# HoangChuongNguyen/cope-nerf

Measured on AMD Instinct MI355X. Metric: rays/sec (train step incl. backward) at 4096 rays × 128 samples, higher is better.
Workload: dtype fp32; 1 GPU; C2: synthetic scene, 4096 rays x 128 samples (64 coarse + 4x16 importance) per GPU, fp32, fixed poses, full train step (fwd + losses + bwd + Adam); rays_per_gpu=4096, samples_per_ray=128, global_rays=4096, hip_graph=False, parallelism=single

## Files before the change

### cope-nerf_amd/copenerf/_lib.py

```python
from __future__ import annotations

import ctypes
import os
import threading

import numpy as np

_HERE = os.path.dirname(os.path.abspath(__file__))
LIB_NAME = "libcopenerf.so"
LIB_PATH = os.environ.get("COPENERF_LIB", os.path.join(_HERE, LIB_NAME))

ABI_VERSION = 21

c_f32p = ctypes.c_void_p
c_i32 = ctypes.c_int32
c_i64 = ctypes.c_int64
c_f32 = ctypes.c_float
c_ptr = ctypes.c_void_p

EPI_STORE = 0
EPI_SOFTPLUS = 1
EPI_RELU = 2
EPI_MUL = 3
EPI_TANGENT = 4
EPI_BWD_SOFTPLUS = 5
EPI_BWD_RELU = 6
EPI_SOFTPLUS_HEAD = 8


class WnJob(ctypes.Structure):
    _fields_ = [("v", c_ptr), ("g", c_ptr), ("w", c_ptr), ("dw", c_ptr), ("dv", c_ptr), ("dg", c_ptr),
                ("rows", c_i32), ("cols", c_i32)]


class LinearDesc(ctypes.Structure):
# ... 320 lines not shown
```

### cope-nerf_amd/copenerf/ops.py

```python
from __future__ import annotations

import ctypes
import math

import torch

from . import _lib
from ._lib import (EPI_BWD_RELU, EPI_BWD_SOFTPLUS, EPI_MUL, EPI_RELU, EPI_SOFTPLUS, EPI_SOFTPLUS_HEAD,
                   EPI_STORE, EPI_TANGENT)

SQRT2 = float(math.sqrt(2.0))


class KernelTimer:

    def __init__(self, detail=False):
        self.records = []
        self.detail = detail
        self.symbols = {}

    def start(self):
        e = torch.cuda.Event(enable_timing=True)
        e.record()
        return e
# ... 125 lines not shown
        rows, cols = (src.shape[1], src.shape[0]) if transpose else (src.shape[0], src.shape[1])
        j = _lib.PackJob()
        j.src, j.dst = src.data_ptr(), dst.data_ptr()
        j.src_ld = src.stride(0)
        x6 = fmt == "bf16x6"
        d_rows, d_cols = (dst.shape[1], 16 * dst.shape[0]) if x6 else (dst.shape[0], dst.shape[1])
        j.dst_ld = d_rows if x6 else d_cols
        j.rows, j.cols = rows, cols
        j.r0, j.r1 = r0, d_rows if r1 is None else r1
        j.c0, j.c1 = c0, d_cols if c1 is None else c1
        j.transpose, j.format = int(transpose), FORMATS[fmt]
        self.jobs.append(j)
        self.keep.append(src)
        return dst

    def run(self):
        if self.jobs:
            arr = (_lib.PackJob * len(self.jobs))(*self.jobs)
            _lib.check(_lib.load().cn_pack_weights(arr, len(self.jobs), _stream()), "cn_pack_weights")
        self.jobs, self.keep = [], []


_TILE_TAGS = {"4, 2, 2, 4, 16, 1, 2": "sq", "4, 2, 1, 4, 32, 1, 2": "tall", "4, 2, 2, 2, 32, 1, 2": "wide",
              "2, 2, 2, 2, 16, 2, 2": "t128", "4, 1, 1, 2, 16, 2, 2": "t1", "4, 2, 2, 4, 32, 1, 2": "sq",
              "2, 2, 2, 2, 64, 2, 1": "t128", "4, 1, 1, 2, 64, 2, 1": "t1"}


def kernel_name(query, d) -> str:
    buf = ctypes.create_string_buffer(256)
    n = query(d, buf, 256)
    if n < 0:
        raise RuntimeError(f"kernel name query failed ({n}): {_lib.load().cn_last_error().decode()}")
    return buf.value.decode()


def _tile_tag(name, tile):
    args = name[name.index("<") + 1:].split(", ")[:7]
    return _TILE_TAGS.get(", ".join(args), tile)


def linear(A, B, N, K, out0, epilogue, *, bias=None, A2=None, K1=None, rowv=None, colv=None, aux0=None,
           aux1=None, aux2=None, out_split=None, nsplit=None, nzero=None, adiv=1.0, odiv=1.0, beta=100.0,
           threshold=20.0, aux_beta=0.0, aux2_scale=0.0, tile=None, M=None, kalg=None, out1=None, head_w=None,
           head_b=None, head_out=None, head_idx=None, out0_b=None, out1_b=None):
    x6 = B.dim() == 3
    if x6 and (B.dtype != torch.bfloat16 or B.shape[2] != 48 or not B.is_contiguous()):
# ... 961 lines not shown
```

### cope-nerf_amd/csrc/cn_gemm.hip

```cpp
#include "cn_mfma.h"

#include <algorithm>
#include <type_traits>
#include <cstdlib>

namespace cn {

struct LinearArgs {
    const float* A;
    const float* A2;
    const float* B;
    const float* bias;
    const float* rowv;
    const float* colv;
    const float* aux0;
    const float* aux1;
    const float* aux2;
    float* out0;
    float* out1;
    float* out_split;
    int lda, lda2, ldb, ld_aux0, ld_aux1, ld_aux2, ld_out0, ld_out1, ld_split;
    int M, N, K, K1, nzero, nsplit, n_tiles_m, n_tiles_n;
    float inv_adiv, inv_odiv, beta, threshold;
    float aux_c;
    float aux2_scale;
    const float* head_w;
    const float* head_b;
    float* head_out;
    const int* head_idx;
    int flags;
    bf16_t* out0_b;
    bf16_t* out1_b;
    int ld_out0_b, ld_out1_b;
};


constexpr int kTblCols = 512;

#ifndef CN_DMA_A_NT
#define CN_DMA_A_NT 0
#endif
template <int WM, int WN, int TM, int TN, int BK, int OCC, int DEPTH, int EPI, bool ROWV, int MODE_>
__global__ void __launch_bounds__(64 * WM * WN, OCC * WM * WN / 4) linear_kernel(LinearArgs p) {
    constexpr int MODE = MODE_ & 3;
    constexpr bool ABF = (MODE_ & 4) != 0;
    constexpr bool AUX0B = (MODE_ & 8) != 0 && (EPI == CN_EPI_BWD_RELU || EPI == CN_EPI_MUL || EPI == CN_EPI_TANGENT ||
                                                EPI == CN_EPI_BWD_SOFTPLUS);
    constexpr bool AUX12B = (MODE_ & 8) != 0 && EPI == CN_EPI_BWD_SOFTPLUS;
    static_assert(!ABF || MODE == 1, "bf16 A images only in the bf16 MFMA mode");
    constexpr bool AX6 = (MODE_ & 16) != 0;
    static_assert(!AX6 || (MODE == 2 && BK == 16), "bf16x6 A images: 16-deep stages of the bf16x6 mode");
    constexpr int NT = 64 * WM * WN;
    const float* const cA = p.A;
    const float* const cB = p.B;
    float* const cOut0 = p.out0;
    const int cN = p.N, cNzero = p.nzero;
    const float cInvOdiv = p.inv_odiv;
    constexpr int BM = 32 * TM * WM;
    constexpr int BN = 32 * TN * WN;
    constexpr bool BF = MODE != 0;
    constexpr int NPL = MODE == 2 ? 3 : 1;
    constexpr int LS = (BF ? NPL * BK / 2 : BK) + (MODE == 2 && BK == 16 ? 12 : 4);
    constexpr int EPA = ABF ? 8 : 4;
    constexpr int ESA = ABF ? 2 : 4;
    constexpr int KC4 = BK / EPA;
    static_assert(NT % KC4 == 0, "staging rows");
    constexpr int RSTEP = NT / KC4;
    constexpr int KCB = BF ? NPL * BK / 8 : BK / 4;
    constexpr int RSTEPB = MODE == 2 ? 1 : NT / KCB;
    static_assert(BM % RSTEP == 0 && (MODE == 2 || (NT % KCB == 0 && BN % RSTEPB == 0)), "tile/thread mismatch");
    constexpr int ALD = AX6 ? (BM * 6 + NT - 1) / NT : BM / RSTEP;
    constexpr int BLD = MODE == 2 ? (BN * KCB + NT - 1) / NT : BN / RSTEPB;
    constexpr int ESZB = BF ? 2 : 4;
    constexpr int PIECES_PL = BK / 8;
    constexpr int CS = BN + 4;
    constexpr int LDS_FLOATS = 2 * BM * LS + 2 * BN * LS;
    constexpr int NPART = (BM * CS <= LDS_FLOATS) ? 1 : ((BM / 2) * CS <= LDS_FLOATS ? 2 : 4);
    static_assert((BM / NPART) * CS <= LDS_FLOATS, "C tile slab must fit in the staging LDS");
    constexpr int PROWS = BM / NPART;

    constexpr bool kHead = EPI == CN_EPI_SOFTPLUS_HEAD;
    constexpr bool kBias = EPI == CN_EPI_STORE || EPI == CN_EPI_SOFTPLUS || EPI == CN_EPI_RELU || kHead;
    constexpr bool kColv = ROWV || kHead;
    constexpr int TBLC = kHead ? 256 : kTblCols;
    constexpr int TBL = (kBias ? TBLC : 0) + (kColv ? TBLC : 0) + (kHead ? TBLC + 4 : 0);
    constexpr bool kDma = ABF && MODE == 1 && TM * TN >= 8 && BK == 32 && OCC == 1 && BM == 256 && BN == 256;
    constexpr int DNS = 4, DROWB = BK * 2, DSIDEA = BM * DROWB, DSTAGE = (BM + BN) * DROWB;
    constexpr int LDS_MAIN = kDma ? DNS * DSTAGE / 4 + 2 * BM : LDS_FLOATS;
    __shared__ __attribute__((aligned(16))) float smem[LDS_MAIN + TBL];
    float* sA = smem;
    float* sB = smem + 2 * BM * LS;
    float* sBias = smem + LDS_MAIN;
    float* sColv = sBias + (kBias ? TBLC : 0);
    float* sHeadW = sColv + (kColv ? TBLC : 0);

    const int tid = threadIdx.x;
    const int lane = tid & 63;
    const int wave = tid >> 6;
    const int wm = wave / WN;
    const int wn = wave % WN;
    const int T = p.n_tiles_n;
    const int ntiles = ((p.n_tiles_m + 7) / 8) * 8 * T;
    const int nk = p.K / BK;

    const int srow = tid / KC4, sc4 = tid % KC4;
    const int srowb = tid / KCB, scb = tid % KCB;
    int voA[ALD], voA2[ALD], voB[BLD];
    int ldsB[BLD];
    int ldsA[AX6 ? ALD : 1];
#pragma unroll
    for (int q = 0; q < ALD; ++q) {
        if constexpr (AX6) {
            const int w = tid + q * NT;
            voA[q] = w < BM * 6 ? w * 16 : 0;
            voA2[q] = 0;
            ldsA[q] = (w / 6) * LS + ((w % 6) >> 1) * (BK / 2) + 4 * (w & 1);
        } else {
            voA[q] = ((srow + q * RSTEP) * p.lda + sc4 * EPA) * ESA;
            voA2[q] = ((srow + q * RSTEP) * p.lda2 + sc4 * EPA) * ESA;
        }
    }
#pragma unroll
    for (int q = 0; q < BLD; ++q) {
        if constexpr (MODE == 2) {
            const int idx = tid + q * NT;
            const int h = idx / (BN * 6), w = idx % (BN * 6);
            voB[q] = idx < BN * KCB ? h * p.ldb * 96 + w * 16 : 0;
            ldsB[q] = (w / 6) * LS + ((w % 6) >> 1) * (BK / 2) + 8 * h + 4 * (w & 1);
        } else {
            voB[q] = (srowb + q * RSTEPB) * p.ldb * ESZB + scb * 16;
        }
    }
    const int lds_a = srow * LS + sc4 * (ABF || !BF ? 4 : 2);
    const int lds_b = srowb * LS + scb * 4;

    floatx4 ra[DEPTH][ALD], rb[DEPTH][BLD];
    auto gload = [&](int set, int kc, int m0, int n0, bool valid) {
        const int k0 = kc * BK;
        const int rows = valid ? min(BM, p.M - m0) : 0;
        const bool second = k0 >= p.K1;
        const char* abase = second ? reinterpret_cast<const char*>(p.A2) + (int64_t)m0 * p.lda2 * ESA
                                   : reinterpret_cast<const char*>(cA) + (int64_t)m0 * p.lda * ESA;
        const int ald = second ? p.lda2 : p.lda;
        const int ak = second ? k0 - p.K1 : k0;
        if constexpr (AX6) {
            const rsrc_t rA = make_view(reinterpret_cast<const float*>(reinterpret_cast<const char*>(cA) +
                                                                       ((int64_t)kc * p.lda + m0) * 96), rows * 96);
#pragma unroll
            for (int q = 0; q < ALD; ++q) ra[set][q] = bload4(rA, voA[q], 0);
        } else {
        const rsrc_t rA = make_view(reinterpret_cast<const float*>(abase), rows * ald * ESA);
#pragma unroll
        for (int q = 0; q < ALD; ++q) ra[set][q] = bload4(rA, second ? voA2[q] : voA[q], ak * ESA);
        }
        const int64_t bofs = MODE == 2 ? ((int64_t)kc * (BK / 16) * p.ldb + n0) * 96 : (int64_t)n0 * p.ldb * ESZB;
        const rsrc_t rB = make_view(reinterpret_cast<const float*>(reinterpret_cast<const char*>(cB) + bofs),
                                    valid ? (MODE == 2 ? ((BK / 16 - 1) * p.ldb + BN) * 96 : BN * p.ldb * ESZB) : 0);
#pragma unroll
        for (int q = 0; q < BLD; ++q) rb[set][q] = bload4(rB, voB[q], MODE == 2 ? 0 : k0 * ESZB);
    };
    auto lstore = [&](int set, int buf, int piece = -1) {
        float* a = sA + buf * BM * LS + lds_a;
        float* b = sB + buf * BN * LS + lds_b;
#pragma unroll
        for (int q = 0; q < ALD; ++q) {
            if (piece >= 0 && piece != q) continue;
            if constexpr (AX6) {
                if (BM * 6 % NT == 0 || tid + q * NT < BM * 6)
                    *reinterpret_cast<floatx4*>(sA + buf * BM * LS + ldsA[q]) = ra[set][q];
            } else if constexpr (MODE == 2) {
                bf16x4 x0, x1, x2;
                split3(ra[set][q], x0, x1, x2);
                *reinterpret_cast<bf16x4*>(a + q * RSTEP * LS) = x0;
                *reinterpret_cast<bf16x4*>(a + q * RSTEP * LS + BK / 2) = x1;
                *reinterpret_cast<bf16x4*>(a + q * RSTEP * LS + BK) = x2;
            } else if constexpr (ABF)
                *reinterpret_cast<floatx4*>(a + q * RSTEP * LS) = ra[set][q];
            else if constexpr (BF)
                *reinterpret_cast<bf16x4*>(a + q * RSTEP * LS) = __builtin_convertvector(ra[set][q], bf16x4);
            else
                *reinterpret_cast<floatx4*>(a + q * RSTEP * LS) = ra[set][q];
        }
#pragma unroll
        for (int q = 0; q < BLD; ++q) {
            if (piece >= 0 && piece != ALD) continue;
            if constexpr (MODE == 2) {
                const int idx = tid + q * NT;
                if (BN * KCB % NT == 0 || idx < BN * KCB)
                    *reinterpret_cast<floatx4*>(sB + buf * BN * LS + ldsB[q]) = rb[set][q];
            } else {
                *reinterpret_cast<floatx4*>(b + q * RSTEPB * LS) = rb[set][q];
            }
        }
    };
    const int ntm8 = ((p.n_tiles_m + 7) / 8) * 8;
    auto coords = [&](int vt, int& tm, int& tn) {
        tile_coords(vt, T, tm, tn);
        if (p.flags & 1) tm = ntm8 - 1 - tm;
    };
    auto next_valid = [&](int vt) {
        for (; vt < ntiles; vt += gridDim.x) {
            int tm, tn;
            coords(vt, tm, tn);
            if (tm * BM < p.M) return vt;
        }
        return ntiles;
    };

    constexpr bool kSeg = MODE == 2 && TM * TN >= 8 && TN > ALD && DEPTH == 2 && OCC == 1 && BK == 16;
    const int arow = wm * TM * 32 + (lane & 31);
    const int brow = wn * TN * 32 + (lane & 31);
    const int kofs = (BK / 2) * (lane >> 5);
    const int Nmain = (EPI == CN_EPI_MUL && p.nsplit < cN) ? p.nsplit : cN;
    constexpr int C4 = BN / 4;
    constexpr int RPP = NT / C4;
    constexpr int GMAX = OCC >= 3 ? 2 : 4;
    constexpr int GROUP = (PROWS / RPP) < GMAX ? (PROWS / RPP) : GMAX;
    static_assert((PROWS / RPP) % GROUP == 0, "epilogue passes");
    constexpr bool kAux0 = EPI == CN_EPI_MUL || EPI == CN_EPI_TANGENT || EPI == CN_EPI_BWD_SOFTPLUS ||
                           EPI == CN_EPI_BWD_RELU;
    constexpr bool kAux1 = EPI == CN_EPI_BWD_SOFTPLUS;

    const int c4 = tid % C4;
    const int rr = tid / C4;
    const int voO0 = (rr * p.ld_out0 + 4 * c4) * 4;
    const int voO1 = (rr * p.ld_out1 + 4 * c4) * 4;
    const int voX0 = (rr * p.ld_aux0 + 4 * c4) * 4;
    const int voX1 = (rr * p.ld_aux1 + 4 * c4) * (AUX12B ? 2 : 4);
    const int voX2 = (rr * p.ld_aux2 + 4 * c4) * (AUX12B ? 2 : 4);
    const int voS = (rr * p.ld_split + 4 * c4) * 4;
    const int voX0b = (rr * p.ld_aux0 + 4 * c4) * 2;
    const int voO0b = (rr * p.ld_out0_b + 4 * c4) * 2;
    const int voO1b = (rr * p.ld_out1_b + 4 * c4) * 2;
    const float c_exp = p.beta * 1.44269504088896341f;
    const float c_thr = p.threshold * 1.44269504088896341f;
    const float c_log = 0.693147180559945309f / p.beta;

    int vt = next_valid(blockIdx.x);
    if (vt >= ntiles) return;
    if constexpr (TBL > 0) {
        const rsrc_t rbias = make_view(p.bias, kBias && p.bias ? cN * 4 : 0);
        const rsrc_t rcolv = make_view(p.colv, kColv && p.colv ? cN * 4 : 0);
        const rsrc_t rhw = make_view(p.head_w, kHead ? cN * 4 : 0);
        for (int i = tid; i < TBLC / 4; i += NT) {
            if (kBias) *reinterpret_cast<floatx4*>(sBias + 4 * i) = bload4(rbias, 16 * i, 0);
            if (kColv) *reinterpret_cast<floatx4*>(sColv + 4 * i) = bload4(rcolv, 16 * i, 0);
            if (kHead) *reinterpret_cast<floatx4*>(sHeadW + 4 * i) = bload4(rhw, 16 * i, 0);
        }
        if (kHead && tid == 0) sHeadW[TBLC] = p.head_b[0];
    }
    int tm, tn;
    coords(vt, tm, tn);

    const uint32_t lds0 = (uint32_t)reinterpret_cast<uintptr_t>((__attribute__((address_space(3))) float*)smem);
    const int dwave = __builtin_amdgcn_readfirstlane(tid >> 6);
    const bool dsb = dwave >= 4;
    const int drow = (dwave & 3) * 64 + (lane >> 2);
    const int dch = (lane & 3) ^ ((lane >> 4) & 3);
    auto ufirst = [](const void* ptr) {
        const uint64_t x = reinterpret_cast<uint64_t>(ptr);
        const uint32_t lo = __builtin_amdgcn_readfirstlane((uint32_t)x), hi = __builtin_amdgcn_readfirstlane((uint32_t)(x >> 32));
        return reinterpret_cast<void*>(((uint64_t)hi << 32) | lo);
// ... 23 lines not shown
                __builtin_amdgcn_raw_ptr_buffer_load_lds(v, (__attribute__((address_space(3))) void*)(dst + j * 1024), 16,
                                                         (drow + 16 * j) * ld * 2 + (kk + dch * 8) * 2, 0, 0, 2);
        } else {
#pragma unroll
            for (int j = 0; j < 4; ++j)
                __builtin_amdgcn_raw_ptr_buffer_load_lds(v, (__attribute__((address_space(3))) void*)(dst + j * 1024), 16,
                                                         (drow + 16 * j) * ld * 2 + (kk + dch * 8) * 2, 0, 0, 0);
        }
    };
    const int dsw = ((lane & 31) >> 2) & 3;
    uint32_t daoff[2], dboff[2];
#pragma unroll
    for (int ks = 0; ks < 2; ++ks) {
        const int ch = ((2 * ks + (lane >> 5)) ^ dsw) << 4;
        daoff[ks] = lds0 + (wm * TM * 32 + (lane & 31)) * DROWB + ch;
        dboff[ks] = lds0 + DSIDEA + (wn * TN * 32 + (lane & 31)) * DROWB + ch;
    }
    if constexpr (kDma) {
        __syncthreads();
#pragma unroll
        for (int d = 0; d < DNS - 1; ++d) dma_issue(d, d, tm * BM, tn * BN, true);
    } else {
#pragma unroll
        for (int d = 0; d < DEPTH; ++d) gload(d, d, tm * BM, tn * BN, true);
#pragma unroll
        for (int d = 0; d < DEPTH; ++d) {
#pragma unroll
            for (int q = 0; q < ALD; ++q) asm volatile("" : "+v"(ra[d][q]));
#pragma unroll
            for (int q = 0; q < BLD; ++q) asm volatile("" : "+v"(rb[d][q]));
        }
    }
    float tbias[TN], tcolv[TN], thw[TN];
    float thb = 0.0f;
#pragma unroll
    for (int j = 0; j < TN; ++j) {
        const int c = min(wn * TN * 32 + (lane & 31) + 32 * j, TBLC - 1);
        tbias[j] = kDma && kBias ? sBias[c] : 0.0f;
        tcolv[j] = kDma && kColv ? sColv[c] : 0.0f;
        thw[j] = kDma && kHead ? sHeadW[c] : 0.0f;
    }
    if (kDma && kHead) thb = sHeadW[TBLC];
    const bool epi_big = !kHead || p.out0 || p.out1 || p.out0_b || p.out1_b;
    constexpr int kRingWait = 4 * (DNS - 2);
    constexpr int kEpiMinVmem = TM * 8 * TN;
    constexpr int kEpiWait = kRingWait + kEpiMinVmem < 63 ? kRingWait + kEpiMinVmem : 63;
    static_assert(!kDma || (kEpiWait > kRingWait && kRingWait + kEpiMinVmem >= kEpiWait),
                  "the epilogue's memory operations must cover the wait past the ring's chunks");
    int gs = 0;
    bool gs_first = true;

    while (vt < ntiles) {
        const int m0 = tm * BM, n0 = tn * BN;
        const int vt_next = next_valid(vt + gridDim.x);
        int tm_next = 0, tn_next = 0;
        if (vt_next < ntiles) coords(vt_next, tm_next, tn_next);

        if constexpr (!kDma) {
            lstore(0, 0);
            __syncthreads();
        }

        floatx16 acc[TM][TN];
#pragma unroll
        for (int i = 0; i < TM; ++i)
#pragma unroll
            for (int j = 0; j < TN; ++j)
#pragma unroll
                for (int r = 0; r < 16; ++r) acc[i][j][r] = 0.0f;

        auto compute = [&](int cur, auto side) {
            if constexpr (MODE == 2) {
                const float* a_base = sA + cur * BM * LS + arow * LS + 4 * (lane >> 5);
                const float* b_base = sB + cur * BN * LS + brow * LS + 4 * (lane >> 5);
                if constexpr (TM * TN >= 8) {
#pragma unroll
                    for (int ks = 0; ks < BK / 16; ++ks) {
                        bf16x8 af[3][TM];
#pragma unroll
                        for (int t = 0; t < 3; ++t)
#pragma unroll
                            for (int i = 0; i < TM; ++i)
                                af[t][i] = *reinterpret_cast<const bf16x8*>(a_base + i * 32 * LS + t * (BK / 2) + ks * 8);
#pragma unroll
                        for (int j = 0; j < TN; ++j) {
                            bf16x8 bj[3];
#pragma unroll
                            for (int t = 0; t < 3; ++t)
                                bj[t] = *reinterpret_cast<const bf16x8*>(b_base + j * 32 * LS + t * (BK / 2) + ks * 8);
                            constexpr int TA[6] = {0, 1, 0, 2, 1, 0};
                            constexpr int TB[6] = {0, 0, 1, 0, 1, 2};
#pragma unroll
                            for (int u = 0; u < 6; ++u)
#pragma unroll
                                for (int i = 0; i < TM; ++i)
                                    acc[i][j] = __builtin_amdgcn_mfma_f32_32x32x16_bf16(af[TA[u]][i], bj[TB[u]], acc[i][j],
                                                                                         0, 0, 0);
// ... 108 lines not shown
                for (int i = 0; i < TM; ++i)
#pragma unroll
                    for (int j = 0; j < TN; ++j)
                        acc[i][j] = __builtin_amdgcn_mfma_f32_32x32x16_bf16(af[1][i], bfr[1][j], acc[i][j], 0, 0, 0);
            }
            gs = (gs + nk) % DNS;
            gs_first = false;
        } else if constexpr (DEPTH == 1) {
            for (int kc = 0; kc < nk; ++kc) {
                const int cur = kc & 1;
                const bool more = kc + 1 < nk;
                gload(0, more ? kc + 1 : 0, more ? m0 : m_next, more ? n0 : n_next, more || has_next);
                compute(cur, [](int) {});
                if (more) lstore(0, cur ^ 1);
                __syncthreads();
            }
        } else {
            static_assert(DEPTH % 2 == 0, "LDS buffer of chunk kc+j is j&1");
            for (int kc = 0; kc < nk; kc += DEPTH) {
#pragma unroll
                for (int j = 0; j < DEPTH; ++j) {
                    const int cn = kc + j + DEPTH;
                    const bool here = cn < nk;
                    gload(j, here ? cn : cn - nk, here ? m0 : m_next, here ? n0 : n_next, here || has_next);
                    if constexpr (kSeg) {
                        compute(j & 1, [&](int jj) {
                            if (jj <= ALD) lstore((j + 1) % DEPTH, (j + 1) & 1, jj);
                        });
                        __syncthreads();
                        continue;
                    }
                    compute(j & 1, [](int) {});
                    if (kc + j + 1 < nk) lstore((j + 1) % DEPTH, (j + 1) & 1);
                    __syncthreads();
                }
            }
        }

        if constexpr (!kDma) {
#pragma unroll
            for (int d = 0; d < DEPTH; ++d) {
#pragma unroll
                for (int q = 0; q < ALD; ++q) asm volatile("" : "+v"(ra[d][q]));
#pragma unroll
                for (int q = 0; q < BLD; ++q) asm volatile("" : "+v"(rb[d][q]));
            }
        }
        const int rows = min(BM, p.M - m0);
        const TileView tO0 = {cOut0 + (int64_t)m0 * p.ld_out0 + n0, p.ld_out0, cOut0 ? (rows * p.ld_out0 - n0) * 4 : 0};
        const TileView tO1 = {p.out1 + (int64_t)m0 * p.ld_out1 + n0, p.ld_out1, p.out1 ? (rows * p.ld_out1 - n0) * 4 : 0};
        const TileView tX0 = AUX0B ? tile_view_b16(p.aux0, p.ld_aux0, m0, n0, rows)
                                  : TileView{p.aux0 + (int64_t)m0 * p.ld_aux0 + n0, p.ld_aux0,
                                             p.aux0 ? (rows * p.ld_aux0 - n0) * 4 : 0};
        const TileView tO0b = tile_view_b16(p.out0_b, p.ld_out0_b, m0, n0, rows);
        const TileView tO1b = tile_view_b16(p.out1_b, p.ld_out1_b, m0, n0, rows);
        const bool has_b0 = MODE == 1 && p.out0_b != nullptr;
        const bool has_b1 = MODE == 1 && p.out1_b != nullptr;
        const bool has_o0 = cOut0 != nullptr, has_o1 = p.out1 != nullptr;
        const TileView tX1 = AUX12B ? tile_view_b16(p.aux1, p.ld_aux1, m0, n0, rows)
                                    : TileView{p.aux1 + (int64_t)m0 * p.ld_aux1 + n0, p.ld_aux1,
                                               p.aux1 ? (rows * p.ld_aux1 - n0) * 4 : 0};
        const TileView tX2 = AUX12B ? tile_view_b16(p.aux2, p.ld_aux2, m0, n0, rows)
                                    : TileView{p.aux2 + (int64_t)m0 * p.ld_aux2 + n0, p.ld_aux2,
                                               p.aux2 ? (rows * p.ld_aux2 - n0) * 4 : 0};
        const TileView tR = {p.rowv + m0, 1, ROWV ? rows * 4 : 0};
        const int sh = n0 - p.nsplit;
        const TileView tS = {p.out_split + (int64_t)m0 * p.ld_split + sh, p.ld_split,
                             p.out_split ? (rows * p.ld_split - sh) * 4 : 0};
// ... 370 lines not shown
                            for (int j = 0; j < TN; ++j) {
                                prev0[j] = ov0[j];
                                prev1[j] = ov1[j];
                            }
                        }
                    }
#pragma unroll
                    for (int off = 16; off > 0; off >>= 1) part += __shfl_xor(part, off, 64);
                    if ((lane & 31) == 0) sRed[(lrow + rowi) * 2 + wn] = part;
                }
            __syncthreads();
            if (tid < BM) {
                const int row = m0 + tid;
                if (row < p.M) {
                    const float sum = sRed[tid * 2] + sRed[tid * 2 + 1];
                    const int dst = p.head_idx ? p.head_idx[row] : row;
                    p.head_out[dst] = sum + (kDma ? thb : sHeadW[TBLC]);
                }
            }
        };
        using T1 = std::true_type;
        using F0 = std::false_type;
        auto run_direct_plain = [&]() {
            if (has_o0) {
                if (has_b0) direct_plain(T1{}, T1{}); else direct_plain(T1{}, F0{});
            } else {
                direct_plain(F0{}, T1{});
            }
        };
        auto run_direct_aux = [&]() {
            auto go = [&](auto spl) {
                if (has_o0) {
                    if (has_b0) direct_aux(T1{}, T1{}, spl); else direct_aux(T1{}, F0{}, spl);
                } else {
                    direct_aux(F0{}, T1{}, spl);
                }
            };
            if constexpr (EPI == CN_EPI_MUL) {
                if (p.nsplit < cN) go(T1{}); else go(F0{});
            } else {
                go(F0{});
            }
        };
        if constexpr (kDirectOnly) {
            if constexpr (kDirectHead) direct_head();
            else if constexpr (kDirectAux) run_direct_aux();
            else run_direct_plain();
        } else {
            if (kDirectAux && tile_main) {
                run_direct_aux();
            } else if (kDirect && tile_main) {
                run_direct_plain();
            } else {
                if (tile_main) passes(std::true_type{});
                else passes(std::false_type{});
// ... 393 lines not shown
}

#ifndef CN_AB_X6_AIMG
#define CN_AB_X6_AIMG 0
#endif

template <int WM, int WN, int TM, int TN, int BK, int OCC, int DEPTH, int MODE = 0>
static int launch_linear_tile(const cn_linear_desc* d, LinearArgs& a, hipStream_t s) {
    if constexpr (MODE == 2 && CN_AB_X6_AIMG && BK == 16 && TM * TN >= 8) {
        if (linear_mode_bits(d, MODE) == 18) return launch_linear_tile_m<WM, WN, TM, TN, BK, OCC, DEPTH, 18>(d, a, s);
    }
    if constexpr (MODE == 1) {
        switch (linear_mode_bits(d, MODE)) {
            case 5: return launch_linear_tile_m<WM, WN, TM, TN, BK, OCC, DEPTH, 5>(d, a, s);
            case 9: return launch_linear_tile_m<WM, WN, TM, TN, BK, OCC, DEPTH, 9>(d, a, s);
            case 13: return launch_linear_tile_m<WM, WN, TM, TN, BK, OCC, DEPTH, 13>(d, a, s);
            default: break;
        }
    }
    return launch_linear_tile_m<WM, WN, TM, TN, BK, OCC, DEPTH, MODE>(d, a, s);
}


enum LinearTile { LT_BF_SQ, LT_BF_T0, LT_BF_T1, LT_X6_SQ, LT_X6_TALL, LT_X6_WIDE, LT_X6_T128, LT_X6_T1, LT_F_T0_D2,
                  LT_F_T0_D1, LT_F_T1_D2, LT_F_T1_D1 };
#define CN_LINEAR_TILES(X)                 \
    X(LT_BF_SQ, 4, 2, 2, 4, 32, 1, 2, 1)   \
    X(LT_BF_T0, 2, 2, 2, 2, 64, 2, 1, 1)   \
    X(LT_BF_T1, 4, 1, 1, 2, 64, 2, 1, 1)   \
    X(LT_X6_SQ, 4, 2, 2, 4, 16, 1, 2, 2)   \
    X(LT_X6_TALL, 4, 2, 1, 4, 32, 1, 2, 2) \
    X(LT_X6_WIDE, 4, 2, 2, 2, 32, 1, 2, 2) \
    X(LT_X6_T128, 2, 2, 2, 2, 16, 2, 2, 2) \
    X(LT_X6_T1, 4, 1, 1, 2, 16, 2, 2, 2)   \
    X(LT_F_T0_D2, 2, 2, 2, 2, 32, 2, 2, 0) \
    X(LT_F_T0_D1, 2, 2, 2, 2, 32, 2, 1, 0) \
    X(LT_F_T1_D2, 4, 1, 1, 2, 32, 2, 2, 0) \
    X(LT_F_T1_D1, 4, 1, 1, 2, 32, 2, 1, 0)

#ifndef CN_AB_X6_BWD_SQ
#define CN_AB_X6_BWD_SQ 0
#endif

#ifndef CN_X6_SMALL_M
#define CN_X6_SMALL_M 0
#endif

static LinearTile choose_linear_tile(const cn_linear_desc* d) {
    const int e = d->epilogue;
    const bool head = e == CN_EPI_SOFTPLUS_HEAD;
    const bool wide_n = d->tile == 0 && d->N > 128 && d->N <= 256 && !d->rowv;
    const bool longk = d->K >= 128;
    if (d->mfma_dtype == CN_MFMA_BF16) {
        if (wide_n && d->K >= 96 && (longk || head)) return LT_BF_SQ;
        return d->tile == 1 ? LT_BF_T1 : LT_BF_T0;
    }
    if (d->mfma_dtype == CN_MFMA_F32_BF16X6) {
        if (d->tile == 1) return LT_X6_T1;
        if (d->tile == 2) return LT_X6_T128;
        if (d->M <= CN_X6_SMALL_M && wide_n && d->K % 64 == 0 && longk && d->ldb >= 256) {
            if (e == CN_EPI_SOFTPLUS) return LT_X6_T128;
            if (head) return LT_X6_TALL;
        }
        if (wide_n && d->K % 32 == 0 && d->ldb >= 256 && (e != CN_EPI_BWD_SOFTPLUS || CN_AB_X6_BWD_SQ) && (longk || head))
            return LT_X6_SQ;
        const bool tall = e == CN_EPI_MUL || e == CN_EPI_TANGENT || head;
        if (d->K % 64 == 0 && tall && d->N > 128 && d->ldb >= 256 && (longk || head)) return LT_X6_TALL;
        const bool light = e == CN_EPI_STORE || e == CN_EPI_SOFTPLUS || e == CN_EPI_RELU || e == CN_EPI_MUL ||
                           e == CN_EPI_TANGENT;
        if (d->K % 64 == 0 && light && longk) return LT_X6_WIDE;
        return LT_X6_T128;
    }
    const bool even = (d->K % 64) == 0;
    if (d->tile == 1) return even ? LT_F_T1_D2 : LT_F_T1_D1;
    return even ? LT_F_T0_D2 : LT_F_T0_D1;
}

static int linear_plan(const cn_linear_desc* d, LinearArgs& a) {
    CN_REQUIRE(d, CN_ERR_ARG, "cn_linear: null desc");
    const bool head = d->epilogue == CN_EPI_SOFTPLUS_HEAD;
    CN_REQUIRE(d->A && d->B && (d->out0 || d->out0_b || head), CN_ERR_ARG, "cn_linear: A, B and out0 (or out0_b) are required");
    CN_REQUIRE(d->M >= 0 && d->N > 0 && d->K > 0, CN_ERR_SHAPE, "cn_linear: bad M/N/K %d/%d/%d", d->M, d->N, d->K);
    CN_REQUIRE(d->mfma_dtype == CN_MFMA_F32 || d->mfma_dtype == CN_MFMA_BF16 || d->mfma_dtype == CN_MFMA_F32_BF16X6,
               CN_ERR_ARG, "cn_linear: bad mfma_dtype %d", d->mfma_dtype);
    const bool bf = d->mfma_dtype == CN_MFMA_BF16;
    const bool x6 = d->mfma_dtype == CN_MFMA_F32_BF16X6;
    CN_REQUIRE(d->K % (bf ? 64 : 32) == 0, CN_ERR_SHAPE, "cn_linear: K=%d must be a multiple of %d", d->K, bf ? 64 : 32);
    CN_REQUIRE(d->tile >= 0 && d->tile <= 2, CN_ERR_ARG, "cn_linear: bad tile %d", d->tile);
    if (x6 && d->a_bf16 && CN_AB_X6_AIMG) {
        CN_REQUIRE(!d->A2 && !d->aux0_bf16 && !d->aux12_bf16 && !d->out0_b && !d->out1_b && d->lda >= d->M &&
                       al16(d->A) && choose_linear_tile(d) == LT_X6_SQ,
                   CN_ERR_UNSUPPORTED, "cn_linear: bf16x6 A images: 256x256 tile, no A2, lda = image rows >= M");
    } else if (d->a_bf16 || d->aux0_bf16 || d->aux12_bf16 || d->out0_b || d->out1_b) {
        CN_REQUIRE(bf, CN_ERR_UNSUPPORTED, "cn_linear: bf16 operand images need mfma_dtype CN_MFMA_BF16");
        CN_REQUIRE(!d->a_bf16 || (d->lda % 8 == 0 && (!d->A2 || d->lda2 % 8 == 0)), CN_ERR_ALIGN,
                   "cn_linear: bf16 A / A2 need lda, lda2 multiples of 8");
        const int e = d->epilogue;
        CN_REQUIRE(!d->aux0_bf16 || ((e == CN_EPI_BWD_RELU || e == CN_EPI_MUL || e == CN_EPI_TANGENT ||
                                      e == CN_EPI_BWD_SOFTPLUS) && d->aux0 && !d->rowv && d->ld_aux0 % 8 == 0),
                   CN_ERR_UNSUPPORTED, "cn_linear: a bf16 aux0 is for MUL / TANGENT / BWD_SOFTPLUS / BWD_RELU "
                   "(no rowv, ld_aux0 % 8 == 0)");
        CN_REQUIRE(!d->aux12_bf16 || (e == CN_EPI_BWD_SOFTPLUS && !d->rowv && d->aux1 && d->aux2 &&
                                      d->ld_aux1 % 8 == 0 && d->ld_aux2 % 8 == 0),
                   CN_ERR_UNSUPPORTED, "cn_linear: bf16 aux1 / aux2 are for BWD_SOFTPLUS (both set, no rowv, "
                   "leading dimensions % 8 == 0)");
        CN_REQUIRE(e != CN_EPI_BWD_SOFTPLUS || !d->aux1 || (d->aux0_bf16 != 0) == (d->aux12_bf16 != 0),
                   CN_ERR_UNSUPPORTED, "cn_linear: BWD_SOFTPLUS's aux0 and aux1 / aux2 are all bf16 images or all fp32");
        CN_REQUIRE(!d->out0_b || (al16(d->out0_b) && d->ld_out0_b % 8 == 0 && d->ld_out0_b < (1 << 20) &&
                                  d->ld_out0_b >= std::max(d->nzero, d->N)),
                   CN_ERR_ALIGN, "cn_linear: out0_b needs 16-byte alignment and ld_out0_b >= nzero, % 8 == 0");
        CN_REQUIRE(!d->out1_b || (d->epilogue == CN_EPI_SOFTPLUS_HEAD && d->colv && d->aux_beta > 0.0f &&
// ... 77 lines not shown
    const float adiv = d->adiv == 0.0f ? 1.0f : d->adiv;
    const float odiv = d->odiv == 0.0f ? 1.0f : d->odiv;
    a.inv_adiv = 1.0f / adiv;
    a.inv_odiv = 1.0f / odiv;
    a.beta = d->beta;
    a.threshold = d->threshold;
    a.out0_b = static_cast<bf16_t*>(d->out0_b);
    a.out1_b = static_cast<bf16_t*>(d->out1_b);
    a.ld_out0_b = (int)d->ld_out0_b;
    a.ld_out1_b = (int)d->ld_out1_b;
    return CN_OK;
}

extern "C" int cn_linear(const cn_linear_desc* d, cn_stream_t stream) {
    LinearArgs a;
    int rc = linear_plan(d, a);
    if (rc || d->M == 0) return rc;
    hipStream_t s = (hipStream_t)stream;
    switch (choose_linear_tile(d)) {
#define CN_TILE_CASE(T, WM, WN, TM, TN, BK, OCC, DEPTH, MODE) \
        case T: return launch_linear_tile<WM, WN, TM, TN, BK, OCC, DEPTH, MODE>(d, a, s);
        CN_LINEAR_TILES(CN_TILE_CASE)
#undef CN_TILE_CASE
    }
    set_error("cn_linear: no tile");
    return CN_ERR_UNSUPPORTED;
}

extern "C" int cn_linear_kernel_name(const cn_linear_desc* d, char* buf, int32_t len) {
    CN_REQUIRE(d && buf && len > 0, CN_ERR_ARG, "cn_linear_kernel_name: null desc / buffer");
    const char* args = "";
    int mode = 0;
    switch (choose_linear_tile(d)) {
#define CN_TILE_NAME(T, WM, WN, TM, TN, BK, OCC, DEPTH, MODE) \
        case T: args = #WM ", " #WN ", " #TM ", " #TN ", " #BK ", " #OCC ", " #DEPTH; mode = linear_mode_bits(d, MODE); break;
        CN_LINEAR_TILES(CN_TILE_NAME)
#undef CN_TILE_NAME
    }
    const int n = snprintf(buf, (size_t)len, "void cn::linear_kernel<%s, %d, %s, %d>(cn::LinearArgs)", args,
                           d->epilogue, d->rowv && (mode & 8) == 0 ? "true" : "false", mode);
    CN_REQUIRE(n < len, CN_ERR_SHAPE, "cn_linear_kernel_name: buffer of %d bytes too small (%d)", len, n + 1);
    return n;
}


extern "C" int cn_row_head(int32_t M, int32_t K, const float* A, int64_t lda, const float* W, int64_t ldw,
                           const float* b, int32_t C, int32_t act, float* out, int64_t ld_out,
                           const int32_t* dst_index, cn_stream_t stream) {
    CN_REQUIRE(A && W && out, CN_ERR_ARG, "cn_row_head: null pointer");
    CN_REQUIRE(K > 0 && K <= 256 && K % 4 == 0 && C >= 1 && C <= 4, CN_ERR_UNSUPPORTED, "cn_row_head: K=%d C=%d", K, C);
    CN_REQUIRE(lda % 4 == 0 && ldw % 4 == 0 && al16(A) && al16(W), CN_ERR_ALIGN, "cn_row_head: alignment");
    CN_REQUIRE(act == 0 || act == 1, CN_ERR_ARG, "cn_row_head: act");
    if (M == 0) return CN_OK;
    const int blocks = std::min(cdiv(M, 32), 8192);
    row_head_kernel<<<blocks, 256, 0, (hipStream_t)stream>>>(M, K, A, lda, W, ldw, b, C, act, out, ld_out, dst_index);
    return check_launch("cn_row_head");
}

extern "C" int cn_scale_cols(int32_t M, int32_t N, const float* X, int64_t ldx, const float* w, const float* rowv,
                             float* out, int64_t ld_out, float act_beta, cn_stream_t stream) {
// ... 122 lines not shown
```

### include/copenerf.h

```cpp
#ifndef COPENERF_H_
#define COPENERF_H_

#include <stddef.h>
#include <stdint.h>

#ifdef __cplusplus
extern "C" {
#endif

#define CN_ABI_VERSION 21

typedef void* cn_stream_t;

typedef enum cn_status {
    CN_OK = 0,
    CN_ERR_ARG = -1,
    CN_ERR_SHAPE = -2,
    CN_ERR_ALIGN = -3,
    CN_ERR_LAUNCH = -4,
    CN_ERR_UNSUPPORTED = -5
} cn_status;

int cn_abi_version(void);
const char* cn_last_error(void);

typedef enum cn_epilogue {
    CN_EPI_STORE = 0,
    CN_EPI_SOFTPLUS = 1,
    CN_EPI_RELU = 2,
    CN_EPI_MUL = 3,
    CN_EPI_TANGENT = 4,
    CN_EPI_BWD_SOFTPLUS = 5,
    CN_EPI_BWD_RELU = 6,
// ... 436 lines not shown
```

Before: 152,100 rays/s.

## Add two-workgroup-per-CU bf16x6 tall tile with single B register set and swizzled LDS

Adds a new bf16x6 GEMM tile (128x256 block, BK 16, occupancy 2). It keeps only one register set for B staging, loading B one k-step ahead instead of DEPTH ahead, and uses a 24-float LDS row stride with an XOR swizzle on the A/B layouts. Together these are meant to fit two workgroups per CU. The tile is selected by default for large-M backward-style epilogues (BWD_SOFTPLUS, MUL, TANGENT, BWD_RELU) with wide N and long K, aiming to hide latency through occupancy. The trade-off is a shallower B prefetch and more complex indexing.

```diff
diff --git a/cope-nerf_amd/copenerf/_lib.py b/cope-nerf_amd/copenerf/_lib.py
--- a/cope-nerf_amd/copenerf/_lib.py
+++ b/cope-nerf_amd/copenerf/_lib.py
@@ -10,7 +10,7 @@
 LIB_NAME = "libcopenerf.so"
 LIB_PATH = os.environ.get("COPENERF_LIB", os.path.join(_HERE, LIB_NAME))
 
-ABI_VERSION = 21
+ABI_VERSION = 22
 
 c_f32p = ctypes.c_void_p
 c_i32 = ctypes.c_int32
diff --git a/cope-nerf_amd/copenerf/ops.py b/cope-nerf_amd/copenerf/ops.py
--- a/cope-nerf_amd/copenerf/ops.py
+++ b/cope-nerf_amd/copenerf/ops.py
@@ -171,6 +171,7 @@
 
 
 _TILE_TAGS = {"4, 2, 2, 4, 16, 1, 2": "sq", "4, 2, 1, 4, 32, 1, 2": "tall", "4, 2, 2, 2, 32, 1, 2": "wide",
+              "2, 2, 2, 4, 16, 2, 2": "tall2",
               "2, 2, 2, 2, 16, 2, 2": "t128", "4, 1, 1, 2, 16, 2, 2": "t1", "4, 2, 2, 4, 32, 1, 2": "sq",
               "2, 2, 2, 2, 64, 2, 1": "t128", "4, 1, 1, 2, 64, 2, 1": "t1"}
 
diff --git a/cope-nerf_amd/csrc/cn_gemm.hip b/cope-nerf_amd/csrc/cn_gemm.hip
--- a/cope-nerf_amd/csrc/cn_gemm.hip
+++ b/cope-nerf_amd/csrc/cn_gemm.hip
@@ -37,6 +37,9 @@
 
 constexpr int kTblCols = 512;
 
+#ifndef CN_AB_TALL2_OFFSET
+#define CN_AB_TALL2_OFFSET 0
+#endif
 #ifndef CN_DMA_A_NT
 #define CN_DMA_A_NT 0
 #endif
@@ -60,7 +63,8 @@
     constexpr int BN = 32 * TN * WN;
     constexpr bool BF = MODE != 0;
     constexpr int NPL = MODE == 2 ? 3 : 1;
-    constexpr int LS = (BF ? NPL * BK / 2 : BK) + (MODE == 2 && BK == 16 ? 12 : 4);
+    constexpr bool kRot = MODE == 2 && BK == 16 && OCC == 2 && TM * TN >= 8 && (MODE_ & 16) == 0;
+    constexpr int LS = kRot ? 24 : (BF ? NPL * BK / 2 : BK) + (MODE == 2 && BK == 16 ? 12 : 4);
     constexpr int EPA = ABF ? 8 : 4;
     constexpr int ESA = ABF ? 2 : 4;
     constexpr int KC4 = BK / EPA;
@@ -87,6 +91,7 @@
     constexpr bool kDma = ABF && MODE == 1 && TM * TN >= 8 && BK == 32 && OCC == 1 && BM == 256 && BN == 256;
     constexpr int DNS = 4, DROWB = BK * 2, DSIDEA = BM * DROWB, DSTAGE = (BM + BN) * DROWB;
     constexpr int LDS_MAIN = kDma ? DNS * DSTAGE / 4 + 2 * BM : LDS_FLOATS;
+    static_assert(!kRot || (LDS_MAIN + TBL) * 4 <= 80 * 1024, "two workgroups per CU: at most 80 KB each");
     __shared__ __attribute__((aligned(16))) float smem[LDS_MAIN + TBL];
     float* sA = smem;
     float* sB = smem + 2 * BM * LS;
@@ -127,15 +132,23 @@
             const int h = idx / (BN * 6), w = idx % (BN * 6);
             voB[q] = idx < BN * KCB ? h * p.ldb * 96 + w * 16 : 0;
             ldsB[q] = (w / 6) * LS + ((w % 6) >> 1) * (BK / 2) + 8 * h + 4 * (w & 1);
+            if constexpr (kRot) {
+                static_assert(!kRot || BN * KCB % NT == 0, "whole pieces per thread");
+                voB[q] = q >= 3 && 3 * NT == 768 ? voB[q - 3] + 128 * 96 : (w / 6) * 96 + ((w % 6) ^ ((w / 6) >> 3 & 1)) * 16;
+                ldsB[q] = idx * 4;
+            }
         } else {
             voB[q] = (srowb + q * RSTEPB) * p.ldb * ESZB + scb * 16;
         }
     }
     const int lds_a = srow * LS + sc4 * (ABF || !BF ? 4 : 2);
+    static_assert(!kRot || RSTEP % 16 == 0, "one exchange bit per thread");
+    const int rotA = ((sc4 >> 1) ^ (srow >> 3 & 1)) * 4 + 2 * (sc4 & 1);
     const int lds_b = srowb * LS + scb * 4;
 
-    floatx4 ra[DEPTH][ALD], rb[DEPTH][BLD];
-    auto gload = [&](int set, int kc, int m0, int n0, bool valid) {
+    constexpr int BSETS = kRot ? 1 : DEPTH;
+    floatx4 ra[DEPTH][ALD], rb[BSETS][BLD];
+    auto gload = [&](int set, int kc, int m0, int n0, bool valid, int what = 0) {
         const int k0 = kc * BK;
         const int rows = valid ? min(BM, p.M - m0) : 0;
         const bool second = k0 >= p.K1;
@@ -143,7 +156,8 @@
                                    : reinterpret_cast<const char*>(cA) + (int64_t)m0 * p.lda * ESA;
         const int ald = second ? p.lda2 : p.lda;
         const int ak = second ? k0 - p.K1 : k0;
-        if constexpr (AX6) {
+        if (what == 2) {
+        } else if constexpr (AX6) {
             const rsrc_t rA = make_view(reinterpret_cast<const float*>(reinterpret_cast<const char*>(cA) +
                                                                        ((int64_t)kc * p.lda + m0) * 96), rows * 96);
 #pragma unroll
@@ -153,11 +167,12 @@
 #pragma unroll
         for (int q = 0; q < ALD; ++q) ra[set][q] = bload4(rA, second ? voA2[q] : voA[q], ak * ESA);
         }
+        if (what == 1) return;
         const int64_t bofs = MODE == 2 ? ((int64_t)kc * (BK / 16) * p.ldb + n0) * 96 : (int64_t)n0 * p.ldb * ESZB;
         const rsrc_t rB = make_view(reinterpret_cast<const float*>(reinterpret_cast<const char*>(cB) + bofs),
                                     valid ? (MODE == 2 ? ((BK / 16 - 1) * p.ldb + BN) * 96 : BN * p.ldb * ESZB) : 0);
 #pragma unroll
-        for (int q = 0; q < BLD; ++q) rb[set][q] = bload4(rB, voB[q], MODE == 2 ? 0 : k0 * ESZB);
+        for (int q = 0; q < BLD; ++q) rb[kRot ? 0 : set][q] = bload4(rB, voB[q], MODE == 2 ? 0 : k0 * ESZB);
     };
     auto lstore = [&](int set, int buf, int piece = -1) {
         float* a = sA + buf * BM * LS + lds_a;
@@ -171,6 +186,13 @@
             } else if constexpr (MODE == 2) {
                 bf16x4 x0, x1, x2;
                 split3(ra[set][q], x0, x1, x2);
+                if constexpr (kRot) {
+                    float* ar = sA + buf * BM * LS + (srow + q * RSTEP) * LS + rotA;
+                    *reinterpret_cast<bf16x4*>(ar) = x0;
+                    *reinterpret_cast<bf16x4*>(ar + BK / 2) = x1;
+                    *reinterpret_cast<bf16x4*>(ar + BK) = x2;
+                    continue;
+                }
                 *reinterpret_cast<bf16x4*>(a + q * RSTEP * LS) = x0;
                 *reinterpret_cast<bf16x4*>(a + q * RSTEP * LS + BK / 2) = x1;
                 *reinterpret_cast<bf16x4*>(a + q * RSTEP * LS + BK) = x2;
@@ -187,7 +209,7 @@
             if constexpr (MODE == 2) {
                 const int idx = tid + q * NT;
                 if (BN * KCB % NT == 0 || idx < BN * KCB)
-                    *reinterpret_cast<floatx4*>(sB + buf * BN * LS + ldsB[q]) = rb[set][q];
+                    *reinterpret_cast<floatx4*>(sB + buf * BN * LS + ldsB[q]) = rb[kRot ? 0 : set][q];
             } else {
                 *reinterpret_cast<floatx4*>(b + q * RSTEPB * LS) = rb[set][q];
             }
@@ -207,7 +229,8 @@
         return ntiles;
     };
 
-    constexpr bool kSeg = MODE == 2 && TM * TN >= 8 && TN > ALD && DEPTH == 2 && OCC == 1 && BK == 16;
+    constexpr bool kSeg = MODE == 2 && TM * TN >= 8 && TN > ALD && DEPTH == 2 && (OCC == 1 || kRot) && BK == 16;
+    const int rotF = ((lane >> 5) ^ ((lane & 31) >> 3 & 1)) * 4;
     const int arow = wm * TM * 32 + (lane & 31);
     const int brow = wn * TN * 32 + (lane & 31);
     const int kofs = (BK / 2) * (lane >> 5);
@@ -238,6 +261,12 @@
 
     int vt = next_valid(blockIdx.x);
     if (vt >= ntiles) return;
+    if constexpr (kRot && CN_AB_TALL2_OFFSET > 0) {
+        if (blockIdx.x >= gridDim.x / 2) {
+            const uint64_t t0 = wall_clock64();
+            while (wall_clock64() - t0 < (uint64_t)CN_AB_TALL2_OFFSET) __builtin_amdgcn_s_sleep(8);
+        }
+    }
     if constexpr (TBL > 0) {
         const rsrc_t rbias = make_view(p.bias, kBias && p.bias ? cN * 4 : 0);
         const rsrc_t rcolv = make_view(p.colv, kColv && p.colv ? cN * 4 : 0);
@@ -307,13 +336,14 @@
         for (int d = 0; d < DNS - 1; ++d) dma_issue(d, d, tm * BM, tn * BN, true);
     } else {
 #pragma unroll
-        for (int d = 0; d < DEPTH; ++d) gload(d, d, tm * BM, tn * BN, true);
+        for (int d = 0; d < DEPTH; ++d) gload(d, d, tm * BM, tn * BN, true, kRot && d > 0 ? 1 : 0);
 #pragma unroll
         for (int d = 0; d < DEPTH; ++d) {
 #pragma unroll
             for (int q = 0; q < ALD; ++q) asm volatile("" : "+v"(ra[d][q]));
 #pragma unroll
-            for (int q = 0; q < BLD; ++q) asm volatile("" : "+v"(rb[d][q]));
+            for (int q = 0; q < BLD; ++q)
+                if (d < BSETS) asm volatile("" : "+v"(rb[d][q]));
         }
     }
     float tbias[TN], tcolv[TN], thw[TN];
@@ -356,8 +386,8 @@
 
         auto compute = [&](int cur, auto side) {
             if constexpr (MODE == 2) {
-                const float* a_base = sA + cur * BM * LS + arow * LS + 4 * (lane >> 5);
-                const float* b_base = sB + cur * BN * LS + brow * LS + 4 * (lane >> 5);
+                const float* a_base = sA + cur * BM * LS + arow * LS + (kRot ? rotF : 4 * (lane >> 5));
+                const float* b_base = sB + cur * BN * LS + brow * LS + (kRot ? rotF : 4 * (lane >> 5));
                 if constexpr (TM * TN >= 8) {
 #pragma unroll
                     for (int ks = 0; ks < BK / 16; ++ks) {
@@ -512,6 +542,19 @@
                 for (int j = 0; j < DEPTH; ++j) {
                     const int cn = kc + j + DEPTH;
                     const bool here = cn < nk;
+                    if constexpr (kRot) {
+                        static_assert(kSeg, "the one-set B staging lives in the pinned segments");
+                        const int cb = kc + j + 1;
+                        const bool hb = cb < nk;
+                        gload(0, hb ? cb : 0, hb ? m0 : m_next, hb ? n0 : n_next, hb || has_next, 2);
+                        gload(j, here ? cn : cn - nk, here ? m0 : m_next, here ? n0 : n_next, here || has_next, 1);
+                        compute(j & 1, [&](int jj) {
+                            if (jj < ALD) lstore((j + 1) % DEPTH, (j + 1) & 1, jj);
+                            if (jj == TN - 1) lstore(0, (j + 1) & 1, ALD);
+                        });
+                        __syncthreads();
+                        continue;
+                    }
                     gload(j, here ? cn : cn - nk, here ? m0 : m_next, here ? n0 : n_next, here || has_next);
                     if constexpr (kSeg) {
                         compute(j & 1, [&](int jj) {
@@ -533,7 +576,8 @@
 #pragma unroll
                 for (int q = 0; q < ALD; ++q) asm volatile("" : "+v"(ra[d][q]));
 #pragma unroll
-                for (int q = 0; q < BLD; ++q) asm volatile("" : "+v"(rb[d][q]));
+                for (int q = 0; q < BLD; ++q)
+                    if (d < BSETS) asm volatile("" : "+v"(rb[d][q]));
             }
         }
         const int rows = min(BM, p.M - m0);
@@ -950,7 +994,7 @@
         using T1 = std::true_type;
         using F0 = std::false_type;
         auto run_direct_plain = [&]() {
-            if (has_o0) {
+            if (has_o0 || kRot) {
                 if (has_b0) direct_plain(T1{}, T1{}); else direct_plain(T1{}, F0{});
             } else {
                 direct_plain(F0{}, T1{});
@@ -958,7 +1002,7 @@
         };
         auto run_direct_aux = [&]() {
             auto go = [&](auto spl) {
-                if (has_o0) {
+                if (has_o0 || kRot) {
                     if (has_b0) direct_aux(T1{}, T1{}, spl); else direct_aux(T1{}, F0{}, spl);
                 } else {
                     direct_aux(F0{}, T1{}, spl);
@@ -1398,13 +1442,14 @@
 }
 
 
-enum LinearTile { LT_BF_SQ, LT_BF_T0, LT_BF_T1, LT_X6_SQ, LT_X6_TALL, LT_X6_WIDE, LT_X6_T128, LT_X6_T1, LT_F_T0_D2,
-                  LT_F_T0_D1, LT_F_T1_D2, LT_F_T1_D1 };
+enum LinearTile { LT_BF_SQ, LT_BF_T0, LT_BF_T1, LT_X6_SQ, LT_X6_TALL2, LT_X6_TALL, LT_X6_WIDE, LT_X6_T128, LT_X6_T1, LT_F_T0_D2,
+                  LT_F_T0_D1, LT_F_T1_D2, LT_F_T1_D1, LT_NONE  };
 #define CN_LINEAR_TILES(X)                 \
     X(LT_BF_SQ, 4, 2, 2, 4, 32, 1, 2, 1)   \
     X(LT_BF_T0, 2, 2, 2, 2, 64, 2, 1, 1)   \
     X(LT_BF_T1, 4, 1, 1, 2, 64, 2, 1, 1)   \
     X(LT_X6_SQ, 4, 2, 2, 4, 16, 1, 2, 2)   \
+    X(LT_X6_TALL2, 2, 2, 2, 4, 16, 2, 2, 2) \
     X(LT_X6_TALL, 4, 2, 1, 4, 32, 1, 2, 2) \
     X(LT_X6_WIDE, 4, 2, 2, 2, 32, 1, 2, 2) \
     X(LT_X6_T128, 2, 2, 2, 2, 16, 2, 2, 2) \
@@ -1414,9 +1459,24 @@
     X(LT_F_T1_D2, 4, 1, 1, 2, 32, 2, 2, 0) \
     X(LT_F_T1_D1, 4, 1, 1, 2, 32, 2, 1, 0)
 
-#ifndef CN_AB_X6_BWD_SQ
-#define CN_AB_X6_BWD_SQ 0
+constexpr int kTall2MinM = 2 * 256 * 128;
+#ifndef CN_X6_TALL2_CLASSES
+#define CN_X6_TALL2_CLASSES ((1u << CN_EPI_BWD_SOFTPLUS) | (1u << CN_EPI_MUL) | (1u << CN_EPI_TANGENT) | (1u << CN_EPI_BWD_RELU))
 #endif
+#ifndef CN_AB_TALL2_ENV
+#define CN_AB_TALL2_ENV 0
+#endif
+static unsigned tall2_classes() {
+#if CN_AB_TALL2_ENV
+    static const unsigned m = [] {
+        const char* e = getenv("COPENERF_TALL2_CLASSES");
+        return e ? (unsigned)strtoul(e, nullptr, 0) : (unsigned)(CN_X6_TALL2_CLASSES);
+    }();
+    return m;
+#else
+    return CN_X6_TALL2_CLASSES;
+#endif
+}
 
 #ifndef CN_X6_SMALL_M
 #define CN_X6_SMALL_M 0
@@ -1434,11 +1494,17 @@
     if (d->mfma_dtype == CN_MFMA_F32_BF16X6) {
         if (d->tile == 1) return LT_X6_T1;
         if (d->tile == 2) return LT_X6_T128;
+        const bool wave_wide = d->N > 128 && d->N <= 256 && !d->rowv && d->K % 32 == 0 && d->ldb >= 256;
+        if (d->tile == 3) return wave_wide ? LT_X6_TALL2 : LT_NONE;
+        if (d->tile == 4) return wave_wide ? LT_X6_SQ : LT_NONE;
         if (d->M <= CN_X6_SMALL_M && wide_n && d->K % 64 == 0 && longk && d->ldb >= 256) {
             if (e == CN_EPI_SOFTPLUS) return LT_X6_T128;
             if (head) return LT_X6_TALL;
         }
-        if (wide_n && d->K % 32 == 0 && d->ldb >= 256 && (e != CN_EPI_BWD_SOFTPLUS || CN_AB_X6_BWD_SQ) && (longk || head))
+        if (wide_n && d->K % 32 == 0 && d->ldb >= 256 && longk && d->M > kTall2MinM && (tall2_classes() >> e & 1) &&
+            !(e == CN_EPI_MUL && d->out_split && d->nsplit < d->N))
+            return LT_X6_TALL2;
+        if (wide_n && d->K % 32 == 0 && d->ldb >= 256 && e != CN_EPI_BWD_SOFTPLUS && (longk || head))
             return LT_X6_SQ;
         const bool tall = e == CN_EPI_MUL || e == CN_EPI_TANGENT || head;
         if (d->K % 64 == 0 && tall && d->N > 128 && d->ldb >= 256 && (longk || head)) return LT_X6_TALL;
@@ -1462,7 +1528,8 @@
     const bool bf = d->mfma_dtype == CN_MFMA_BF16;
     const bool x6 = d->mfma_dtype == CN_MFMA_F32_BF16X6;
     CN_REQUIRE(d->K % (bf ? 64 : 32) == 0, CN_ERR_SHAPE, "cn_linear: K=%d must be a multiple of %d", d->K, bf ? 64 : 32);
-    CN_REQUIRE(d->tile >= 0 && d->tile <= 2, CN_ERR_ARG, "cn_linear: bad tile %d", d->tile);
+    CN_REQUIRE(d->tile >= 0 && d->tile <= 4, CN_ERR_ARG, "cn_linear: bad tile %d", d->tile);
+    CN_REQUIRE(d->tile <= 2 || x6, CN_ERR_UNSUPPORTED, "cn_linear: tile %d is a bf16x6 tile", d->tile);
     if (x6 && d->a_bf16 && CN_AB_X6_AIMG) {
         CN_REQUIRE(!d->A2 && !d->aux0_bf16 && !d->aux12_bf16 && !d->out0_b && !d->out1_b && d->lda >= d->M &&
                        al16(d->A) && choose_linear_tile(d) == LT_X6_SQ,
@@ -1586,13 +1653,17 @@
         case T: return launch_linear_tile<WM, WN, TM, TN, BK, OCC, DEPTH, MODE>(d, a, s);
         CN_LINEAR_TILES(CN_TILE_CASE)
 #undef CN_TILE_CASE
-    }
-    set_error("cn_linear: no tile");
+        case LT_NONE: break;
+    }
+    set_error("cn_linear: tile %d is not built for this descriptor (128 < N <= 256, no rowv, K %% 32 == 0, ldb >= 256)", d->tile);
     return CN_ERR_UNSUPPORTED;
 }
 
 extern "C" int cn_linear_kernel_name(const cn_linear_desc* d, char* buf, int32_t len) {
     CN_REQUIRE(d && buf && len > 0, CN_ERR_ARG, "cn_linear_kernel_name: null desc / buffer");
+    CN_REQUIRE(d->tile >= 0 && d->tile <= 4, CN_ERR_ARG, "cn_linear_kernel_name: bad tile %d", d->tile);
+    CN_REQUIRE(d->tile <= 2 || d->mfma_dtype == CN_MFMA_F32_BF16X6, CN_ERR_UNSUPPORTED,
+               "cn_linear_kernel_name: tile %d is a bf16x6 tile", d->tile);
     const char* args = "";
     int mode = 0;
     switch (choose_linear_tile(d)) {
@@ -1600,6 +1671,9 @@
         case T: args = #WM ", " #WN ", " #TM ", " #TN ", " #BK ", " #OCC ", " #DEPTH; mode = linear_mode_bits(d, MODE); break;
         CN_LINEAR_TILES(CN_TILE_NAME)
 #undef CN_TILE_NAME
+        case LT_NONE:
+            set_error("cn_linear_kernel_name: tile %d is not built for this descriptor", d->tile);
+            return CN_ERR_UNSUPPORTED;
     }
     const int n = snprintf(buf, (size_t)len, "void cn::linear_kernel<%s, %d, %s, %d>(cn::LinearArgs)", args,
                            d->epilogue, d->rowv && (mode & 8) == 0 ? "true" : "false", mode);
diff --git a/include/copenerf.h b/include/copenerf.h
--- a/include/copenerf.h
+++ b/include/copenerf.h
@@ -8,7 +8,7 @@
 extern "C" {
 #endif
 
-#define CN_ABI_VERSION 21
+#define CN_ABI_VERSION 22
 
 typedef void* cn_stream_t;
 
```

After: 154,900 rays/s, median of 6. 1.02x the previous value.
